# hrbigelow/lb-wavenet

Measured on AMD Instinct MI355X. Metric: audio samples/sec: train fwd+bwd & cached autoregressive gen, 1/2/4/8 GPU, higher is better.
Workload: dtype f32; 1 GPU; C2: train step fwd+xent+bwd+TF1-Adam, par/arch3.json (5x10 layers, res/dil 32, skip/post 512, Q 256), B=8 streams x T=4096 per GPU; arch=arch3.json, batch_per_gpu=8, global_batch=8, slice_sz=4096, parallelism=dp1, world_size_seen=1

## Files before the change

lb-wavenet_amd/csrc/gemm.hip:

```cpp
#include <type_traits>
#include <stdlib.h>
#include <string.h>

#include <algorithm>

#include "common.h"
#include "kernels.h"
#include "prologue.h"

namespace {

constexpr int NT = 256;
constexpr int MNPAD = 8;

template <bool KC, int BMN, int BK>
struct Stage {
  static constexpr int SREG = BK * BMN / (4 * NT);
  static constexpr int KCS = BK + 4;
  static constexpr int RS = BMN + MNPAD;
  floatx4 v[SREG];
  static constexpr int LDS_FLOATS = KC ? BMN * KCS : BK * RS;

  LBWN_DEV void load(const float* __restrict__ P, long ld, int mn0, int MN, int k0, int K, int tid,
                     bool , const int* codes = nullptr) {
// ... 650 lines not shown
        if (g.accumulate) v += cv[r];
      }
      if (row < g.M) {
        if (g.c_chain_ls)
          C[(col >> 5) * g.c_chain_ls + ((((long)(row >> 5) * 4 + ((col >> 3) & 3)) * 32 + (row & 31)) * 8 + (col & 7))] = v;
        else
          C[(long)row * g.ldc + col] = v;
        cs[ni] += v;
      }
    }
  }
  if (g.colpart && !raw) {
    float* red = (float*)smem;
#pragma unroll
    for (int ni = 0; ni < NI; ++ni) {
      cs[ni] += __shfl_xor(cs[ni], 32);
      if (h == 0) red[wave * BN + ni * 32 + ci] = cs[ni];
    }
    __syncthreads();
    const int col = n0 + tid;
    if (tid < BN && col < g.N) {
      float s = 0.f;
      for (int w = 0; w < 8; ++w) s += red[w * BN + tid];
      g.colpart[(long)(m0 >> 8) * g.N + col] = s;
    }
  }
}

template <int CTRL>
LBWN_DEV float quad_xor(float v) {
  return __int_as_float(__builtin_amdgcn_update_dpp(0, __float_as_int(v), CTRL, 0xF, 0xF, true));
}

template <int NB, bool AMN = false, bool KL = false>
__global__ __launch_bounds__(512, 1) void gemm_x3q_kernel(lbwn_gemm_args g) {
  static_assert(!KL || AMN, "k_live: the weight-gradient form");
  constexpr int NP = NB == 10 ? 5 : 2;
  constexpr int NTHR = 512, BM = 256, BN = 16 * NB, NH = NB / NP;
  constexpr int SLOT = BN * X3Q_ROW;
  __shared__ __attribute__((aligned(16))) unsigned short smem[2 * SLOT];

  const int tid = threadIdx.x, lane = tid & 63, wave = tid >> 6;
  const int tiles_n = (g.N + BN - 1) / BN;
  if (g.step_advance && blockIdx.x == 0 && blockIdx.y == 0 && blockIdx.z == 0 && tid == 0)
    __hip_atomic_fetch_add(g.step_advance, 1LL, __ATOMIC_RELAXED, __HIP_MEMORY_SCOPE_AGENT);
  const int t = (NB == 10 && g.xcd2d) ? xcd2d_tile((g.M + BM - 1) / BM, tiles_n) : gemm_tile();
  const int m0 = (t / tiles_n) * BM, n0 = (t % tiles_n) * BN;
  const long mw = ((long)t * 8 + wave) * 64 + lane;
  constexpr bool MB = NB == 8 && !AMN;
  const bool bits_in = MB && g.split_stride == 0 && g.mbits, bits_out = MB && g.split_stride == 0 && g.mbits_out;
  const unsigned long long mbr = bits_in ? g.mbits[mw] : 0ull;
  const int kz0 = KL ? 0 : gemm_split() * g.k_per_split;
  const int kz1 = min(g.K, kz0 + g.k_per_split);
  const LiveSlice ls = KL ? live_slice(g) : LiveSlice{0, 0};
  const int* kl = g.k_live + ls.first;
  const bool dead = !AMN && g.row_live && live_ld(g.row_live + (m0 >> 8)) == 0;
  const int ntiles = KL ? ls.n : (dead ? 0 : (kz1 - kz0) / X3_BK);
  const int last = max(ntiles - 1, 0);
  auto kidx = [&](int i) { return KL ? live_ld(kl + i) : i; };

  floatx4 acc[2][NB];
#pragma unroll
  for (int a = 0; a < 2; ++a)
#pragma unroll
    for (int b = 0; b < NB; ++b) acc[a][b] = (floatx4){0.f, 0.f, 0.f, 0.f};

  const int fr = lane & 15, fq = lane >> 4;
  const long aks = g.a_kstride ? g.a_kstride : X3_BK;
  const int ag0 = min(m0 + 32 * wave, max((g.M - 1) & ~31, 0));
  const float* pa0 = AMN ? (g.a_gstride ? g.A + (ag0 >> 5) * g.a_gstride + fr + (long)(kz0 + 8 * fq) * 32
                                        : g.A + min(m0 + 32 * wave + fr, g.M - 1) + (long)(kz0 + 8 * fq) * g.lda)
                         : g.A + (long)min(m0 + 32 * wave + fr, g.M - 1) * g.lda + (kz0 / X3_BK) * aks + 8 * fq;
  const float* pa1 = AMN ? (g.a_gstride ? pa0 + 16
// ... 3 lines not shown
  floatx4 av[2][4];
  auto a_load = [&](auto sset, int kt) {
    constexpr int S = decltype(sset)::value;
    if (AMN) {
      const long ko = (long)kt * X3_BK * g.lda;
#pragma unroll
      for (int j = 0; j < 8; ++j) {
        av[S][j >> 2][j & 3] = pa0[ko + j * g.lda];
        av[S][2 + (j >> 2)][j & 3] = pa1[ko + j * g.lda];
      }
    } else if (NB == 10) {
      av[S][0] = __builtin_nontemporal_load((const floatx4*)(pa0 + kt * aks));
      av[S][1] = __builtin_nontemporal_load((const floatx4*)(pa0 + kt * aks + 4));
      av[S][2] = __builtin_nontemporal_load((const floatx4*)(pa1 + kt * aks));
      av[S][3] = __builtin_nontemporal_load((const floatx4*)(pa1 + kt * aks + 4));
    } else {
      av[S][0] = *(const floatx4*)(pa0 + kt * aks);
      av[S][1] = *(const floatx4*)(pa0 + kt * aks + 4);
      av[S][2] = *(const floatx4*)(pa1 + kt * aks);
      av[S][3] = *(const floatx4*)(pa1 + kt * aks + 4);
    }
  };
  auto a_split = [&](auto sset, int mi, bf16x8 (&f)[3]) {
    constexpr int S = decltype(sset)::value;
    floatx4 x = av[S][2 * mi], y = av[S][2 * mi + 1];
#pragma unroll
    for (int j = 0; j < 4; ++j) {
      x[j] = __int_as_float(max(__float_as_int(x[j]), alo));
      y[j] = __int_as_float(max(__float_as_int(y[j]), alo));
    }
    split8(x, y, f);
  };

  X3Pre<BN, NTHR, X3Q_ROW> sp;
  X3Stage<false, true, BN, NTHR, X3Q_ROW> sm_b;
  auto b_load = [&](auto sset, int kt) {
    constexpr int S = decltype(sset)::value;
    if (AMN) sm_b.template load<S>(kt, 0);
    else sp.template load<S>(kt);
  };
  auto b_store = [&](auto sset, unsigned short* lds) {
    constexpr int S = decltype(sset)::value;
    if (AMN) sm_b.template store<S>(lds, tid, false);
    else sp.template store<S>(lds);
  };
  if (AMN) sm_b.init(g.B, g.ldb, n0, g.N, kz0, tid);
  else sp.init(g.b3, g.K / X3_BK, n0, g.N, kz0, tid);
  int kn = 0;
  if (ntiles > 0) {
    const int k0 = kidx(0), k1 = kidx(min(1, last)), k2 = kidx(min(2, last));
    if (KL) kn = kidx(min(3, last));
    b_load(std::integral_constant<int, 0>(), k0);
    b_store(std::integral_constant<int, 0>(), smem);
    a_load(std::integral_constant<int, 0>(), k0);
    a_load(std::integral_constant<int, 1>(), k1);
    b_load(std::integral_constant<int, 1>(), k1);
    b_load(std::integral_constant<int, 0>(), k2);
  }
  __syncthreads();
  const int fb_off = fr * X3Q_ROW + 8 * fq;

  auto b_frags = [&](const unsigned short* base, int half, bf16x8 (&f)[NH][3]) {
#pragma unroll
    for (int p = 0; p < 3; ++p)
#pragma unroll
      for (int nb = 0; nb < NH; ++nb) f[nb][p] = *(const bf16x8*)(base + fb_off + (NH * half + nb) * 16 * X3Q_ROW + 32 * p);
  };
  auto mfmas = [&](const bf16x8 (&fa)[2][3], const bf16x8 (&fb)[NH][3], int half) {
#pragma unroll
    for (int qq = 0; qq < 6; ++qq) {
      constexpr int PA[6] = {2, 1, 0, 1, 0, 0}, PB[6] = {0, 1, 2, 0, 1, 0};
#pragma unroll
      for (int mi = 0; mi < 2; ++mi)
#pragma unroll
        for (int nb = 0; nb < NH; ++nb)
          acc[mi][NH * half + nb] =
              __builtin_amdgcn_mfma_f32_16x16x32_bf16(fa[mi][PA[qq]], fb[nb][PB[qq]], acc[mi][NH * half + nb], 0, 0, 0);
    }
  };
  bf16x8 fa[2][3];
  auto step = [&](int kt, auto sset) {
    constexpr int S = decltype(sset)::value;
    const unsigned short* cur = smem + (S ^ 1) * SLOT;
    unsigned short* nxt = smem + S * SLOT;
    bf16x8 fn[2][3], fb[NH][3];
    b_frags(cur, 0, fb);
    mfmas(fa, fb, 0);
    a_split(std::integral_constant<int, S>(), 0, fn[0]);
    a_split(std::integral_constant<int, S>(), 1, fn[1]);
    const int k3 = KL ? kn : min(kt + 3, last);
    a_load(std::integral_constant<int, S>(), k3);
    b_store(std::integral_constant<int, S>(), nxt);
    b_load(std::integral_constant<int, S>(), k3);
    if (KL) kn = live_ld(kl + min(kt + 4, last));
#pragma unroll
    for (int part = 1; part < NP; ++part) {
      b_frags(cur, part, fb);
      mfmas(fa, fb, part);
    }
#pragma unroll
    for (int c = 0; c < 2; ++c)
#pragma unroll
      for (int p = 0; p < 3; ++p) fa[c][p] = fn[c][p];
    __syncthreads();
  };
  if (ntiles > 0) {
    a_split(std::integral_constant<int, 0>(), 0, fa[0]);
    a_split(std::integral_constant<int, 0>(), 1, fa[1]);
    a_load(std::integral_constant<int, 0>(), kidx(min(2, last)));
  }
  int kt = 0;
  for (; kt + 1 < ntiles; kt += 2) {
    step(kt, std::integral_constant<int, 1>());
    step(kt + 1, std::integral_constant<int, 0>());
  }
  if (kt < ntiles) step(kt, std::integral_constant<int, 1>());

  float* C = g.C + (long)gemm_split() * g.split_stride;
  const bool raw = g.split_stride != 0;
  const int rbase = m0 + 32 * wave;
  float cs[NB];
  if (g.c_chain_ls && !raw) {
#pragma unroll
    for (int nb = 0; nb < NB; ++nb) {
      cs[nb] = 0.f;
      const int col0 = n0 + nb * 16;
      if (col0 >= g.N) continue;
      const long chunk = g.c_chain_ls * 4;
      const __amdgpu_buffer_rsrc_t rc = __builtin_amdgcn_make_buffer_rsrc(
          C + (long)(col0 >> 5) * g.c_chain_ls, (short)0, (int)(chunk < 0x7fffffffL ? chunk : 0x7fffffffL), 0x00020000);
      const int c = fr & 3, colq = col0 + 4 * (fr >> 2);
#pragma unroll
      for (int mi = 0; mi < 2; ++mi) {
        float a0 = acc[mi][nb][0], a1 = acc[mi][nb][1], a2 = acc[mi][nb][2], a3 = acc[mi][nb][3];
#pragma unroll
        for (int e = 0; e < 4; ++e)
          if (rbase + 16 * mi + 4 * fq + e < g.M) cs[nb] += acc[mi][nb][e];
        const bool odd = c & 1, hi = c & 2;
        {
          const float r0 = quad_xor<0xB1>(odd ? a0 : a1), r1 = quad_xor<0xB1>(odd ? a2 : a3);
          if (odd) { a0 = r0; a2 = r1; } else { a1 = r0; a3 = r1; }
        }
        {
          const float q0 = quad_xor<0x4E>(hi ? a0 : a2), q1 = quad_xor<0x4E>(hi ? a1 : a3);
          if (hi) { a0 = q0; a1 = q1; } else { a2 = q0; a3 = q1; }
        }
        const int row = rbase + 16 * mi + 4 * fq + c;
        const int off = row < g.M ? (int)(((((long)(row >> 5) * 4 + ((colq >> 3) & 3)) * 32 + (row & 31)) * 8 + (colq & 7)) * 4)
                                  : 0x7ffffff0;
// ... 82 lines not shown
        if (g.accumulate) v += cv[e];
      }
      if (col >= g.N) continue;
      if (row < g.M) {
        if (g.c_chain_ls)
          C[(col >> 5) * g.c_chain_ls + ((((long)(row >> 5) * 4 + ((col >> 3) & 3)) * 32 + (row & 31)) * 8 + (col & 7))] = v;
        else
          C[(long)row * g.ldc + col] = v;
        cs[nb] += v;
      }
    }
  }
  if (bits_out) g.mbits_out[mw] = mbw;
  }
  if (g.colpart && !raw) {
    float* red = (float*)smem;
#pragma unroll
    for (int nb = 0; nb < NB; ++nb) {
      cs[nb] += __shfl_xor(cs[nb], 16);
      cs[nb] += __shfl_xor(cs[nb], 32);
      if (fq == 0) red[wave * BN + nb * 16 + fr] = cs[nb];
    }
    __syncthreads();
    const int col = n0 + tid;
    if (tid < BN && col < g.N) {
      float s = 0.f;
      for (int w = 0; w < 8; ++w) s += red[w * BN + tid];
      g.colpart[(long)(m0 >> 8) * g.N + col] = s;
    }
  }
}

static_assert(PLANE_BK == X3_BK, "pre-split chunk = GEMM k-step");
__global__ void split_planes_kernel(SplitJobs jb) { split_planes_body(jb, blockIdx.y, blockIdx.x, gridDim.x); }

}

namespace {
thread_local const char* g_last_form = "";

int gemm_setup(const lbwn_gemm_args& a, int a_kcontig, int b_kcontig, int& split_k, float* slab_ws, int BK,
               int BM, int BN, lbwn_gemm_args& g, dim3& grid) {
  LBWN_REQUIRE(a.M > 0 && a.N > 0 && a.K > 0, "gemm: empty shape M=%d N=%d K=%d", a.M, a.N, a.K);
  LBWN_REQUIRE(a.K % 4 == 0 || !a_kcontig, "gemm: K %% 4 != 0 with k-contiguous A");
  LBWN_REQUIRE(a.K % 4 == 0 || !b_kcontig, "gemm: K %% 4 != 0 with k-contiguous B");
  LBWN_REQUIRE(a.M % 4 == 0 || a_kcontig, "gemm: M %% 4 != 0 with m-contiguous A");
  LBWN_REQUIRE(a.N % 4 == 0, "gemm: N %% 4 != 0");
  LBWN_REQUIRE(a.lda % 4 == 0 && a.ldb % 4 == 0, "gemm: lda/ldb must be multiples of 4");
  LBWN_REQUIRE(a.a_codes == nullptr || !a_kcontig, "gemm: one-hot A must be m-contiguous");
  LBWN_REQUIRE((a.a_codes || (((uintptr_t)a.A) & 15) == 0) && (((uintptr_t)a.B) & 15) == 0,
               "gemm: A/B not 16-B aligned");
  LBWN_REQUIRE(!a.a_kstride || (a_kcontig && a.lda == 32 && a.K % 32 == 0 && !a.a_codes && lbwn_gemm_mode() == 1),
               "gemm: k-blocked A needs k-contiguous A, lda = 32, K %% 32 == 0 and the bf16-split form");
  LBWN_REQUIRE(!a.b_gstride || (!b_kcontig && a.ldb == 32 && !a.b3 && lbwn_gemm_mode() == 1),
               "gemm: mn-blocked B needs mn-contiguous B, ldb = 32, no pre-split and the bf16-split form");
  LBWN_REQUIRE(!a.a_gstride || (!a_kcontig && a.lda == 32 && !b_kcontig && !a.b_gstride && !a.b3 && a.M >= 256 &&
                                a.K % 32 == 0 && !a.mask && !a.bias && !a.colpart && !a.c_chain_ls && !a.a_codes &&
                                lbwn_gemm_mode() == 1),
               "gemm: mn-blocked A needs the AMN weight-gradient form (lda = 32, M >= 256, K %% 32 == 0)");
  LBWN_REQUIRE(!a.splits_deferred || (!a.bias && !a.relu_out && !a.mask && !a.accumulate),
               "gemm: deferred split-K needs a plain product");
  if (split_k < 1) split_k = 1;
  g = a;
  int kps = (a.K + split_k - 1) / split_k;
  kps = (kps + BK - 1) / BK * BK;
  split_k = (a.K + kps - 1) / kps;
  g.k_per_split = kps;
// ... 65 lines not shown
                   !(X3Q && X3R && a_kcontig && a.b3 && (a.colpart || (a.N <= 2048 && (a.M >= 8192 || a.row_exact)))),
               "gemm (bf16 split): chain-order C on the A-in-registers form (gemm_x3q_kernel) takes no bias / relu_out / "
               "mask bits");
  LBWN_REQUIRE(!(a.mbits || a.mbits_out) ||
                   (lbwn_gemm_x3q8_form(a.M, a.N, a.K, a_kcontig, a.b3 != nullptr, a.row_exact, a.colpart != nullptr) &&
                    split_k <= 1),
               "gemm (bf16 split): mask bits need the gemm_x3q_kernel<8> form without split-K");
  LBWN_REQUIRE(!a.row_live || (lbwn_gemm_row_live_form(a.M, a.N, a.K, a_kcontig, a.b3 != nullptr, a.row_exact,
                                                       a.colpart != nullptr) && split_k <= 1),
               "gemm (bf16 split): row_live needs the k-contiguous gemm_x3q_kernel<8 / 10> form without split-K");
  const bool klist = a.k_live || a.nk_live || a.k_pre;
  LBWN_REQUIRE(!klist || (a.k_live && a.nk_live && a.k_pre && !a_kcontig && !b_kcontig && !a.b3 && !a.a_gstride && !a.b_gstride &&
                          !a.colpart && !a.c_chain_ls && lbwn_gemm_k_live_form(a.M, a.N, a.K)),
               "gemm (bf16 split): k_live needs a plain mn-contiguous weight-gradient product with K %% 32 == 0");
  const int wm = (a.colpart || (a_kcontig && a.N <= 2048 && (a.M >= 8192 || a.row_exact))) ? 4 : 2;
  lbwn_gemm_args g;
  dim3 grid;
  int e = gemm_setup(a, a_kcontig, b_kcontig, split_k, slab_ws, X3_BK, 64 * wm, 128, g, grid);
  if (e) return e;
  const bool kfull = a.K % X3_BK == 0, pre = a.b3 != nullptr;
  if (X3Q && !a_kcontig && !b_kcontig && kfull && !pre && !a.mask && !a.bias && !a.colpart && !a.c_chain_ls &&
      !a.b_gstride && a.M >= 256 && a.N % 4 == 0 && (((a.M + 255) / 256) * ((a.N + 127) / 128) >= 8 || a.a_gstride)) {
    if ((e = gemm_setup(a, a_kcontig, b_kcontig, split_k, slab_ws, X3_BK, 256, a.N <= 96 ? 96 : 128, g, grid))) return e;
    g_last_form = a.N <= 96 ? "x3q<6,amn>" : klist ? "x3q<8,amn,kl>" : "x3q<8,amn>";
    if (a.N <= 96) gemm_x3q_kernel<6, true><<<grid, 512, 0, st>>>(g);
    else if (klist) gemm_x3q_kernel<8, true, true><<<grid, 512, 0, st>>>(g);
    else gemm_x3q_kernel<8, true><<<grid, 512, 0, st>>>(g);
    LBWN_CHECK_LAUNCH();
    return splitk_finish(a, split_k, slab_ws, st);
  }
  LBWN_REQUIRE(!a.a_gstride, "gemm: mn-blocked A (a_gstride) needs the AMN A-in-registers form (X3Q, no pre-split B, "
                             "no epilogue, M >= 256)");
  if (wm == 4 && X3R && kfull && pre && a_kcontig) {
    if (a.N <= 96) {
      grid.x = (unsigned)(((a.M + 255) / 256) * ((a.N + 95) / 96));
      g_last_form = X3Q ? "x3q<6>" : "x3r<3>";
      if (X3Q) gemm_x3q_kernel<6><<<grid, 512, 0, st>>>(g);
      else gemm_x3r_kernel<3><<<grid, 512, 0, st>>>(g);
    } else if (X3Q && a.N % 160 == 0 && a.N > 512) {
      grid.x = (unsigned)(((a.M + 255) / 256) * (a.N / 160));
      g_last_form = "x3q<10>";
      gemm_x3q_kernel<10><<<grid, 512, 0, st>>>(g);
    } else if (X3Q) {
      g_last_form = "x3q<8>";
      gemm_x3q_kernel<8><<<grid, 512, 0, st>>>(g);
    } else {
      g_last_form = "x3r<4>";
      gemm_x3r_kernel<4><<<grid, 512, 0, st>>>(g);
    }
    LBWN_CHECK_LAUNCH();
  } else if (wm == 4) {
    if (kfull && pre) e = gemm_launch_x3_t<true, true, 4>(g, grid, a_kcontig, b_kcontig, st);
    else if (kfull) e = gemm_launch_x3_t<true, false, 4>(g, grid, a_kcontig, b_kcontig, st);
    else e = gemm_launch_x3_t<false, false, 4>(g, grid, a_kcontig, b_kcontig, st);
  } else if (klist) {
    g_last_form = "x3<kl>";
    gemm_x3_kernel<false, false, true, false, 2, 1, true><<<grid, 256, 0, st>>>(g);
    LBWN_CHECK_LAUNCH();
  } else {
    if (kfull && pre) e = gemm_launch_x3_t<true, true, 2>(g, grid, a_kcontig, b_kcontig, st);
    else if (kfull) e = gemm_launch_x3_t<true, false, 2>(g, grid, a_kcontig, b_kcontig, st);
    else e = gemm_launch_x3_t<false, false, 2>(g, grid, a_kcontig, b_kcontig, st);
  }
  if (e) return e;
  return splitk_finish(a, split_k, slab_ws, st);
}

template <int BK, int BMT, int BNT>
int gemm_launch_t(const lbwn_gemm_args& a, int a_kcontig, int b_kcontig, int split_k, float* slab_ws, hipStream_t st) {
  lbwn_gemm_args g;
  dim3 grid;
  int e = gemm_setup(a, a_kcontig, b_kcontig, split_k, slab_ws, BK, BMT, BNT, g, grid);
  if (e) return e;
  g_last_form = a_kcontig ? (b_kcontig ? "f32<akc,bkc>" : "f32<akc,bmn>") : (b_kcontig ? "f32<amn,bkc>" : "f32<amn,bmn>");
  if (a_kcontig && b_kcontig) gemm_f32_kernel<true, true, BK, BMT, BNT><<<grid, NT, 0, st>>>(g);
  else if (a_kcontig) gemm_f32_kernel<true, false, BK, BMT, BNT><<<grid, NT, 0, st>>>(g);
  else if (b_kcontig) gemm_f32_kernel<false, true, BK, BMT, BNT><<<grid, NT, 0, st>>>(g);
  else gemm_f32_kernel<false, false, BK, BMT, BNT><<<grid, NT, 0, st>>>(g);
// ... 68 lines not shown
```

lb-wavenet_amd/csrc/engine.cpp:

```cpp
#include <stdio.h>
#include <stdlib.h>
#include <string.h>

#include <algorithm>
#include <new>

#include "../../include/lbwn.h"
#include "common.h"
#include "kernels.h"

struct lbwn_plan {
  int chain_xcd = 0;
  int dz_xcd2d = 1;
  int fwd_mode = -1;
  int ncu = 0;
  size_t oMBS = 0, oMBR = 0;
  bool mb_s = false, mb_r = false;
  bool mbits_ok = true;
  size_t oLIVE = 0;
  bool skip_ok = true;
  bool live_valid = false;
  bool dv_blk = false;
  bool dz_blk = false;
  int head_colparts = 0;
// ... 415 lines not shown
    p->oPADG = carve(cur, sizeof(float) * hp);
  }
  p->total = cur;
  *out = p;
  return 0;
}

void lbwn_plan_destroy(lbwn_plan* p) { delete p; }

int lbwn_plan_tensor(const lbwn_plan* p, const char* name, size_t* off, size_t* bytes) {
  LBWN_REQUIRE(p && name && off && bytes, "plan_tensor: null argument");
  const size_t M = (size_t)p->M, f = sizeof(float);
  if (!strcmp(name, "x")) { *off = p->oX; *bytes = f * (size_t)p->x_layer_stride * p->L; }
  else if (!strcmp(name, "z")) { *off = p->oZ; *bytes = f * M * p->L * p->Cd; }
  else if (!strcmp(name, "s")) { *off = p->oS; *bytes = f * M * p->Cs; }
  else if (!strcmp(name, "r2")) { *off = p->oR2; *bytes = f * M * p->Cp; }
  else if (!strcmp(name, "logits")) { *off = p->oLOG; *bytes = f * M * p->Q; }
  else if (!strcmp(name, "status")) { *off = p->oSTATUS; *bytes = 16; }
  else if (!strcmp(name, "ctrace")) { *off = p->oCTRACE; *bytes = 8 * 2 * 16 * (size_t)p->a.n_blocks * p->a.n_block_layers; }
  else if (!strcmp(name, "dh")) { *off = p->oDH; *bytes = f * M * p->Cp; }
  else if (!strcmp(name, "ds")) { *off = p->oDS; *bytes = f * M * p->Cs; }
  else if (!strcmp(name, "dz")) { *off = p->oDZ; *bytes = f * (p->dz_blk ? (size_t)m32(p->M) : M) * p->L * p->Cd; }
  else if (!strcmp(name, "tlive")) { *off = p->oLIVE; *bytes = 4 * ((M + 255) / 256); }
  else if (!strcmp(name, "klive")) { *off = p->oLIVE + 4 * ((M + 255) / 256); *bytes = 4 * ((M + 31) / 32); }
  else if (!strcmp(name, "nklive")) { *off = p->oLIVE + 4 * ((M + 255) / 256 + (M + 31) / 32); *bytes = 4; }
  else if (!strcmp(name, "kpre")) { *off = p->oLIVE + 4 * ((M + 255) / 256 + (M + 31) / 32 + 1); *bytes = 4 * ((M + 31) / 32 + 1); }
  else if (!strcmp(name, "cond") && p->Lo) { *off = p->oCOND; *bytes = f * M * 2 * p->L * p->Cd; }
  else if (!strcmp(name, "dvall") && p->Lo) {
    *off = p->oDVALL;
    *bytes = f * (p->dv_blk ? (size_t)m32(p->M) : M) * 2 * p->L * p->Cd;
  }
  else if (!strcmp(name, "gctab") && p->Ge) { *off = p->oGCTAB; *bytes = f * p->ncat1 * 2 * p->L * p->Cd; }
  else if (!strcmp(name, "gcd") && p->Ge) { *off = p->oGCD; *bytes = f * p->ncat1 * 2 * p->L * p->Cd; }
  else LBWN_REQUIRE(false, "plan_tensor: unknown tensor '%s'", name);
  return 0;
}
size_t lbwn_plan_workspace_bytes(const lbwn_plan* p) { return p ? p->total : 0; }

int lbwn_plan_info(const lbwn_plan* p, const char* key, int64_t* value) {
  LBWN_REQUIRE(p && key && value, "plan_info: null argument");
  if (!strcmp(key, "up_fused")) *value = p->up_fused;
  else if (!strcmp(key, "up_fused_bwd")) *value = p->up_fused_bwd;
  else if (!strcmp(key, "lc_in_chain")) *value = p->oLCX != 0 && p->chain;
  else if (!strcmp(key, "split_dlc")) *value = p->split_dlc;
  else if (!strcmp(key, "split_dlcx")) *value = p->split_dlcx;
  else if (!strcmp(key, "split_dlct")) *value = p->split_dlct;
  else if (!strncmp(key, "split_up", 8) && key[8] >= '0' && key[8] <= '7' && !key[9])
    *value = p->split_up[key[8] - '0'];
  else if (!strcmp(key, "dv_blk")) *value = p->dv_blk;
  else if (!strcmp(key, "dlc_parts")) *value = p->dlc_parts;
  else if (!strcmp(key, "dmel_fused")) *value = p->dmel_fused;
  else LBWN_REQUIRE(false, "plan_info: unknown key '%s'", key);
  return 0;
}

static int* live_t(const lbwn_plan* p, void* ws) { return reinterpret_cast<int*>(static_cast<char*>(ws) + p->oLIVE); }
static int* live_k(const lbwn_plan* p, void* ws) { return live_t(p, ws) + (p->M + 255) / 256; }
static int* live_n(const lbwn_plan* p, void* ws) { return live_k(p, ws) + (p->M + 31) / 32; }
static int* live_p(const lbwn_plan* p, void* ws) { return live_n(p, ws) + 1; }

static const unsigned short* w3(const lbwn_plan* p, void* ws, int i) {
  return (p->oW3[i] && lbwn_gemm_mode() == 1) ? reinterpret_cast<const unsigned short*>(static_cast<char*>(ws) + p->oW3[i])
                                              : nullptr;
}

static lbwn_gemm_args gemm0() {
// ... 745 lines not shown
```

lb-wavenet_amd/csrc/pack.hip:

```cpp
#include <string.h>

#include "common.h"
#include "kernels.h"
#include "layer_common.h"
#include "prologue.h"

namespace {


__global__ void pack_layers_kernel(const float* sig, const float* gate, const float* sig_b, const float* gate_b,
                                   const float* res, const float* res_b, float* out, int Cr, int Cd) {
  const int l = blockIdx.x;
  const float* ws = sig + (long)l * 2 * Cr * Cd;
  const float* wg = gate + (long)l * 2 * Cr * Cd;
  const float* wr = res + (long)l * Cd * Cr;
  float* img = out + (long)l * WIMG;
  for (int e = threadIdx.x; e < 64 * WS; e += blockDim.x) {
    const int k = e / WS, o = e % WS;
    const int tap = k >> 5, in = k & 31, oc = o & 31;
    float v = 0.f;
    if (o < 64 && in < Cr && oc < Cd) v = (o < 32 ? ws : wg)[(tap * Cr + in) * Cd + oc];
    img[e] = v;
  }
  for (int e = threadIdx.x; e < 32 * XS; e += blockDim.x) {
// ... 165 lines not shown
  const int nlc = lcout ? L : 0;
  if (l < L) {
    pack_x3_body(l, sig, gate, sig_b, gate_b, res, res_b, fout, Cr, Cd);
  } else if (l < 2 * L) {
    pack_bx3_body(l - L, sig, gate, res, bout, Cr, Cd);
  } else if (l < 2 * L + nlc) {
    if (lc16) pack_lc16_body(l - 2 * L, lc_sig, lc_gate, lcout, Lo, Cd);
    else pack_lc_x3_body(l - 2 * L, lc_sig, lc_gate, lcout, Lo, Cd);
  } else {
    const int n = (l - 2 * L - nlc) * 256 + threadIdx.x;
    if (n < Cs) {
      float s = 0.f;
#pragma unroll 10
      for (int k = 0; k < L; ++k) s += skip_b[(long)k * Cs + n];
      bsum[n] = s;
    }
  }
}
__global__ __launch_bounds__(256) void pack_layers_fb_x3_kernel(const float* sig, const float* gate,
                                                                const float* sig_b, const float* gate_b,
                                                                const float* res, const float* res_b,
                                                                unsigned short* fout, float* bout, int L, int Cr,
                                                                int Cd, const float* skip_b, int Cs, float* bsum,
                                                                const float* lc_sig, const float* lc_gate, int Lo,
                                                                unsigned short* lcout, int lc16) {
  pack_fb_x3_block(blockIdx.x, sig, gate, sig_b, gate_b, res, res_b, fout, bout, L, Cr, Cd, skip_b, Cs, bsum, lc_sig,
                   lc_gate, Lo, lcout, lc16);
}

struct PrologueK {
  lbwn_prologue_args a;
  SplitJobs jb;
  int nz, ns, ne, nd, np;
  int nl;
  bool ev4, dv4;
};
__global__ __launch_bounds__(256) void step_prologue_kernel(PrologueK k) {
  const lbwn_prologue_args& a = k.a;
  long b = blockIdx.x;
  if (b < k.nl) {
    live_lists_body(a.ids, a.B, a.T, a.tlive, a.klive, a.nklive, a.kpre);
    return;
  }
  b -= k.nl;
  if (b < (long)k.ns * a.njobs) {
    split_planes_body(k.jb, (int)(b / k.ns), b % k.ns, k.ns);
    return;
  }
  b -= (long)k.ns * a.njobs;
  if (b < k.ne) {
    embed_flat_body(b, k.ne, a.q, a.pre, a.pre_b, a.X, a.B, a.T, a.H, a.Cr, a.Q, k.ev4);
    return;
  }
  b -= k.ne;
  if (b < k.nd) {
    dsep_flat_body<true>(b, k.nd, a.X, a.xls, const_cast<float*>(a.save), a.L, a.nbl, a.B, a.T, a.H, a.Cr, k.dv4);
    return;
  }
  b -= k.nd;
  if (b < k.nz) {
    zero_body(b, k.nz, (unsigned*)a.zero, (long)(a.zero_bytes / 4));
    return;
  }
  b -= k.nz;
  pack_fb_x3_block((int)b, a.sig, a.gate, a.sig_b, a.gate_b, a.res, a.res_b, a.fout, a.bout, a.L, a.Cr, a.Cd,
                   a.skip_b, a.Cs, a.bsum, a.lc_sig, a.lc_gate, a.Lo, a.lcout, a.lc16);
}

}

int lbwn_layer_image_floats() { return WIMG; }
int lbwn_layer_image_x3_elems() { return XIMG_US; }
int lbwn_lc_image_x3_elems() { return LCIMG_US; }
int lbwn_lc_image16_elems() { return LC16IMG_US; }
int lbwn_lc_in_chain_ok(int Lo) { return Lo > 16 * (LC_K - 1) && Lo <= LC_KP && Lo % 4 == 0; }
int lbwn_layer_image_bx3_floats() { return BIMG_F; }

int lbwn_pack_layers_launch(const float* sig, const float* gate, const float* sig_b, const float* gate_b,
                            const float* res, const float* res_b, float* out, int L, int Cr, int Cd, hipStream_t st) {
  pack_layers_kernel<<<L, 256, 0, st>>>(sig, gate, sig_b, gate_b, res, res_b, out, Cr, Cd);
  LBWN_CHECK_LAUNCH();
  return 0;
}

int lbwn_pack_layers_fb_x3_launch(const float* sig, const float* gate, const float* sig_b, const float* gate_b,
                                  const float* res, const float* res_b, unsigned short* fout, float* bout, int L,
                                  int Cr, int Cd, const float* skip_b, int Cs, float* bsum, const float* lc_sig,
                                  const float* lc_gate, int Lo, unsigned short* lcout, hipStream_t st, int lc16) {
  LBWN_REQUIRE(Cr <= 32 && Cd <= 32 && (((uintptr_t)fout) & 15) == 0 && (((uintptr_t)bout) & 15) == 0,
               "pack_layers_fb_x3: bad arguments");
  LBWN_REQUIRE(!lcout || (lc_sig && lc_gate && Lo >= 1 && Lo <= LC_KP && (((uintptr_t)lcout) & 15) == 0),
               "pack_layers_fb_x3: bad LC image arguments");
  const int nsum = (skip_b && bsum) ? (Cs + 255) / 256 : 0;
  const int nlc = lcout ? L : 0;
  pack_layers_fb_x3_kernel<<<2 * L + nlc + nsum, 256, 0, st>>>(sig, gate, sig_b, gate_b, res, res_b, fout, bout, L, Cr,
                                                               Cd, skip_b, Cs, bsum, lc_sig, lc_gate, Lo, lcout,
                                                               lc16);
  LBWN_CHECK_LAUNCH();
  return 0;
}
int lbwn_step_prologue_launch(const lbwn_prologue_args& a, hipStream_t st) {
  LBWN_REQUIRE(a.Cr <= 32 && a.Cd <= 32 && (((uintptr_t)a.fout) & 15) == 0 && (((uintptr_t)a.bout) & 15) == 0,
               "step_prologue: bad pack arguments");
  LBWN_REQUIRE(!a.lcout || (a.lc_sig && a.lc_gate && a.Lo >= 1 && a.Lo <= LC_KP && (((uintptr_t)a.lcout) & 15) == 0),
               "step_prologue: bad LC image arguments");
  LBWN_REQUIRE(a.njobs >= 0 && a.njobs <= 6 && a.zero_bytes % 4 == 0 && a.q && a.pre && a.X && a.save,
               "step_prologue: bad arguments");
  PrologueK k;
  memset(&k, 0, sizeof(k));
  k.a = a;
  long most = 0;
  for (int j = 0; j < a.njobs; ++j) {
    LBWN_REQUIRE(a.W[j] && a.out[j] && a.rows[j] > 0 && a.K[j] > 0, "step_prologue: bad split job");
    k.jb.W[j] = a.W[j]; k.jb.ldw[j] = a.ldw[j]; k.jb.rows[j] = a.rows[j]; k.jb.K[j] = a.K[j];
    k.jb.trans[j] = a.trans[j]; k.jb.out[j] = a.out[j];
    most = std::max(most, (long)a.rows[j] * ((a.K[j] + PLANE_BK - 1) / PLANE_BK) * (PLANE_BK / 2));
  }
  auto blocks = [](long n, long per, long cap) { return (int)std::max(1L, std::min(cap, (n + per - 1) / per)); };
  k.ns = blocks(most, 1024, 256);
  LBWN_REQUIRE((long)a.B * a.T * a.Cr < (1L << 31) && (long)dsep_rows(a.L, a.nbl, 1) * a.B * a.Cr < (1L << 31),
               "step_prologue: x / SAVE exceed 32-bit indexing");
  k.ev4 = embed_v4(a.pre, a.pre_b, a.X, a.Cr);
  k.dv4 = dsep_v4(a.X, a.xls, a.save, a.Cr);
  k.ne = blocks((long)a.B * a.T * (k.ev4 ? a.Cr / 4 : a.Cr), 256, 2048);
  k.nd = blocks((long)dsep_rows(a.L, a.nbl, a.B) * (k.dv4 ? a.Cr / 4 : a.Cr), 256, 2048);
  k.nz = a.zero_bytes ? blocks((long)(a.zero_bytes / 4), 1024, 256) : 0;
  k.np = 2 * a.L + (a.lcout ? a.L : 0) + ((a.skip_b && a.bsum) ? (a.Cs + 255) / 256 : 0);
  LBWN_REQUIRE(!a.ids || (a.tlive && a.klive && a.nklive && a.kpre), "step_prologue: bad live-list arguments");
  k.nl = a.ids ? 1 : 0;
  const long grid = (long)k.nl + (long)k.ns * a.njobs + k.ne + k.nd + k.nz + k.np;
  step_prologue_kernel<<<(unsigned)grid, 256, 0, st>>>(k);
  LBWN_CHECK_LAUNCH();
  return 0;
}
```

lb-wavenet_amd/csrc/prologue.h:

```cpp
#pragma once
#include "common.h"

constexpr int PLANE_BK = 32;

__host__ __device__ inline int dsep_rows(int L, int nbl, int B) {
  return ((L / nbl) * ((1 << nbl) - 1) + ((1 << (L % nbl)) - 1)) * B;
}

template <bool TO_X>
LBWN_DEV void dsep_flat_body(long blk, long nblk, float* xall, long xls, float* save, int L, int nbl, int B, int T,
                             int H, int Cr, bool v4) {
  const int per = (1 << nbl) - 1, rows = dsep_rows(L, nbl, B);
  const int cw = v4 ? Cr >> 2 : Cr;
  const int n = rows * cw;
  for (int e = (int)(blk * 256) + (int)threadIdx.x; e < n; e += (int)(nblk * 256)) {
    const int R = e / cw, c = e - R * cw;
    const int run = R / (B * per), w = R - run * (B * per);
    const int k = 31 - __builtin_clz(w / B + 1);
    const int local = w - B * ((1 << k) - 1);
    const int b = local >> k, i = local & ((1 << k) - 1), d = 1 << k;
    float* xr = xall + (long)(run * nbl + k) * xls + ((long)b * (H + T) + (TO_X ? H - d + i : H + T - d + i)) * Cr;
    float* sv = save + (long)R * Cr;
    if (v4) {
      if (TO_X) *(floatx4*)(xr + 4 * c) = *(const floatx4*)(sv + 4 * c);
// ... 9 lines not shown
inline bool dsep_v4(const float* xall, long xls, const float* save, int Cr) {
  return (Cr & 3) == 0 && (xls & 3) == 0 && al16(xall) && al16(save);
}
inline bool embed_v4(const float* pre, const float* pre_b, const float* x0, int Cr) {
  return (Cr & 3) == 0 && al16(pre) && (!pre_b || al16(pre_b)) && al16(x0);
}

LBWN_DEV void embed_flat_body(long blk, long nblk, const int* __restrict__ q, const float* __restrict__ pre,
                              const float* pre_b, float* x0, int B, int T, int H, int Cr, int Q, bool v4) {
  const int cw = v4 ? Cr >> 2 : Cr;
  const int n = B * T * cw;
  for (int e = (int)(blk * 256) + (int)threadIdx.x; e < n; e += (int)(nblk * 256)) {
    const int m = e / cw, c = e - m * cw;
    const int b = m / T, t = m - b * T;
    int code = q[m];
    code = code < 0 ? 0 : (code >= Q ? Q - 1 : code);
    float* xo = x0 + ((long)b * (H + T) + H + t) * Cr;
    if (v4) {
      floatx4 v = *(const floatx4*)(pre + (long)code * Cr + 4 * c);
      if (pre_b) v += *(const floatx4*)(pre_b + 4 * c);
      *(floatx4*)(xo + 4 * c) = v;
    } else {
      float v = pre[(long)code * Cr + c];
      if (pre_b) v += pre_b[c];
      xo[c] = v;
    }
  }
}

LBWN_DEV void zero_body(long blk, long nblk, unsigned* p, long n) {
  for (long e = blk * 256 + threadIdx.x; e < n; e += nblk * 256) p[e] = 0u;
}

LBWN_DEV void live_lists_body(const int* __restrict__ ids, int B, int T, int* tlive, int* klive, int* nklive,
                              int* kpre) {
  __shared__ int wcnt[4];
  const int M = B * T, nk = (M + 31) / 32, nt = (M + 255) / 256;
  const int tid = threadIdx.x, lane = tid & 63, w = tid >> 6;
  const int inc = 64 % T;
  constexpr int NL = 16, KW = 2 * NL, KR = 4 * KW;
  auto row0 = [&](int k0) { return 32 * (k0 + KW * w) + lane; };
  int v[NL], nx[NL];
  auto load = [&](int (&d)[NL], int k0) {
#pragma unroll
    for (int j = 0; j < NL; ++j) d[j] = ids[min(row0(k0) + 64 * j + 1, M - 1)];
  };
  load(v, 0);
  int base = 0;
  for (int k0 = 0; k0 < nk; k0 += KR) {
    load(nx, min(k0 + KR, nk));
    const int r0 = row0(k0);
    int t = r0 % T;
    unsigned live = 0u;
#pragma unroll
    for (int j = 0; j < NL; ++j) {
      const unsigned long long bal = __ballot((r0 + 64 * j < M) & (t != T - 1) & (v[j] != 0));
      live |= (unsigned)((unsigned)bal != 0u) << (2 * j);
      live |= (unsigned)((bal >> 32) != 0ull) << (2 * j + 1);
      t += inc;
      t -= t >= T ? T : 0;
    }
    const int k = k0 + KW * w + lane;
    if (lane == 0) wcnt[w] = __popc(live);
    __syncthreads();
    int off = base, tot = 0;
#pragma unroll
    for (int i = 0; i < 4; ++i) {
      off += i < w ? wcnt[i] : 0;
      tot += wcnt[i];
    }
    const int pos = off + __popc(live & ((1u << (lane & 31)) - 1u));
    if (lane < KW && k < nk) kpre[k] = pos;
    if (lane < KW && ((live >> lane) & 1u)) klive[pos] = k;
    if (lane < KW && (lane & 7) == 0 && (k >> 3) < nt) tlive[k >> 3] = ((live >> lane) & 0xffu) != 0u;
    base += tot;
    __syncthreads();
#pragma unroll
    for (int j = 0; j < NL; ++j) v[j] = nx[j];
  }
  if (tid == 0) {
    *nklive = base;
    kpre[nk] = base;
  }
}

struct SplitJobs {
  const float* W[6];
  long ldw[6];
  int rows[6], K[6], trans[6];
  unsigned short* out[6];
};
LBWN_DEV void split_planes_body(const SplitJobs& jb, int jj, long blk, long nblk) {
  const float* __restrict__ W = jb.W[jj];
  const long ldw = jb.ldw[jj];
  const int rows = jb.rows[jj], K = jb.K[jj], trans = jb.trans[jj];
  unsigned short* __restrict__ out = jb.out[jj];
  const int kch = (K + PLANE_BK - 1) / PLANE_BK;
  const long total = (long)rows * kch * (PLANE_BK / 2);
  for (long e = blk * 256 + threadIdx.x; e < total; e += nblk * 256) {
    const int j2 = (int)(e % (PLANE_BK / 2)) * 2;
    const long rc = e / (PLANE_BK / 2);
    const int kc = (int)(rc % kch), r = (int)(rc / kch);
    const int k = kc * PLANE_BK + j2;
    floatx2 x;
    x[0] = k < K ? (trans ? W[(long)k * ldw + r] : W[(long)r * ldw + k]) : 0.f;
    x[1] = k + 1 < K ? (trans ? W[(long)(k + 1) * ldw + r] : W[(long)r * ldw + k + 1]) : 0.f;
    unsigned h, m, l;
    split2(x, h, m, l);
    unsigned* o = (unsigned*)(out + rc * (3 * PLANE_BK) + j2);
    o[0] = h;
    o[PLANE_BK / 2] = m;
    o[PLANE_BK] = l;
  }
}
```

Measured before the change: 17.86 million audio samples/s.

## Load pre-split B tiles via global_load_lds DMA with four-slot LDS ring

Adds a DMA variant of the x3q GEMM kernel in which B tiles are copied straight from global memory into LDS with global_load_lds_dwordx4, bypassing the register-staged load/store path. It uses a four-slot LDS ring, issues DMA for two tiles ahead every other step, and replaces per-step __syncthreads with explicit vmcnt/lgkmcnt waits plus a barrier every two steps. The goal is to cut VGPR pressure and store instructions for B and to overlap loads with MFMA work. This DMA variant is now the default for the NB=8 pre-split path and opt-in via env var for the NB=6 and NB=10 paths. It doubles LDS use and depends on hand-written waitcnt counts being exact.

After: 17.90 million audio samples/s (median of 3 runs). About the same (+0.2%).

```diff
diff --git a/lb-wavenet_amd/csrc/gemm.hip b/lb-wavenet_amd/csrc/gemm.hip
--- a/lb-wavenet_amd/csrc/gemm.hip
+++ b/lb-wavenet_amd/csrc/gemm.hip
@@ -706,13 +706,23 @@
   return __int_as_float(__builtin_amdgcn_update_dpp(0, __float_as_int(v), CTRL, 0xF, 0xF, true));
 }
 
-template <int NB, bool AMN = false, bool KL = false>
+LBWN_DEV void x3q_dma16(const unsigned short* sbase, unsigned voff, unsigned lds_dst) {
+  unsigned saved;
+  asm volatile("s_mov_b32 %0, m0\n\ts_mov_b32 m0, %1\n\ts_nop 0\n\tglobal_load_lds_dwordx4 %2, %3\n\ts_mov_b32 m0, %0"
+               : "=&s"(saved)
+               : "s"(lds_dst), "v"(voff), "s"(sbase)
+               : "memory");
+}
+
+template <int NB, bool AMN = false, bool KL = false, bool DMA = false>
 __global__ __launch_bounds__(512, 1) void gemm_x3q_kernel(lbwn_gemm_args g) {
   static_assert(!KL || AMN, "k_live: the weight-gradient form");
+  static_assert(!DMA || !AMN, "B by LDS-DMA: the pre-split k-contiguous forms");
   constexpr int NP = NB == 10 ? 5 : 2;
   constexpr int NTHR = 512, BM = 256, BN = 16 * NB, NH = NB / NP;
   constexpr int SLOT = BN * X3Q_ROW;
-  __shared__ __attribute__((aligned(16))) unsigned short smem[2 * SLOT];
+  constexpr int NSLOT = DMA ? 4 : 2;
+  __shared__ __attribute__((aligned(16))) unsigned short smem[NSLOT * SLOT];
 
   const int tid = threadIdx.x, lane = tid & 63, wave = tid >> 6;
   const int tiles_n = (g.N + BN - 1) / BN;
@@ -782,6 +792,29 @@
     split8(x, y, f);
   };
 
+  constexpr int NPIECE = BN * 14 / 64, PW = (NPIECE + 7) / 8;
+  static_assert((BN * 14) % 64 == 0, "B by LDS-DMA: whole 1-KiB pieces");
+  const int wv = __builtin_amdgcn_readfirstlane(wave);
+  unsigned dvoff[PW];
+  const unsigned short* dbase = nullptr;
+  unsigned ddst = 0;
+  if (DMA) {
+    const int kchunks = g.K / X3_BK;
+#pragma unroll
+    for (int i = 0; i < PW; ++i) {
+      const int gi = min(wv + 8 * i, NPIECE - 1) * 64 + lane, r = gi / 14, part = gi % 14;
+      dvoff[i] = (unsigned)(((long)min(n0 + r, g.N - 1) * kchunks * (3 * X3_BK) + 8 * (part < 12 ? part : 0)) * 2);
+    }
+    dbase = g.b3 + (long)(kz0 / X3_BK) * (3 * X3_BK);
+    ddst = (unsigned)(uintptr_t)(__attribute__((address_space(3))) unsigned short*)smem + wv * 1024;
+  }
+  auto b_dma = [&](int kt) {
+    const unsigned short* sb = dbase + (long)min(kt, last) * (3 * X3_BK);
+    const unsigned dst = ddst + (kt & 3) * (SLOT * 2);
+#pragma unroll
+    for (int i = 0; i < PW; ++i) x3q_dma16(sb, dvoff[i], dst + min(8 * i, NPIECE - 1 - wv) * 1024);
+  };
+
   X3Pre<BN, NTHR, X3Q_ROW> sp;
   X3Stage<false, true, BN, NTHR, X3Q_ROW> sm_b;
   auto b_load = [&](auto sset, int kt) {
@@ -795,9 +828,17 @@
     else sp.template store<S>(lds);
   };
   if (AMN) sm_b.init(g.B, g.ldb, n0, g.N, kz0, tid);
-  else sp.init(g.b3, g.K / X3_BK, n0, g.N, kz0, tid);
+  else if (!DMA) sp.init(g.b3, g.K / X3_BK, n0, g.N, kz0, tid);
   int kn = 0;
-  if (ntiles > 0) {
+  if (DMA) {
+    if (ntiles > 0) {
+      b_dma(0);
+      b_dma(1);
+      a_load(std::integral_constant<int, 0>(), 0);
+      a_load(std::integral_constant<int, 1>(), min(1, last));
+    }
+    asm volatile("s_waitcnt vmcnt(8)\n\ts_waitcnt lgkmcnt(0)\n\ts_barrier" ::: "memory");
+  } else if (ntiles > 0) {
     const int k0 = kidx(0), k1 = kidx(min(1, last)), k2 = kidx(min(2, last));
     if (KL) kn = kidx(min(3, last));
     b_load(std::integral_constant<int, 0>(), k0);
@@ -807,7 +848,7 @@
     b_load(std::integral_constant<int, 1>(), k1);
     b_load(std::integral_constant<int, 0>(), k2);
   }
-  __syncthreads();
+  if (!DMA) __syncthreads();
   const int fb_off = fr * X3Q_ROW + 8 * fq;
 
   auto b_frags = [&](const unsigned short* base, int half, bf16x8 (&f)[NH][3]) {
@@ -831,28 +872,51 @@
   bf16x8 fa[2][3];
   auto step = [&](int kt, auto sset) {
     constexpr int S = decltype(sset)::value;
-    const unsigned short* cur = smem + (S ^ 1) * SLOT;
+    const unsigned short* cur = smem + (DMA ? (kt & 3) : (S ^ 1)) * SLOT;
     unsigned short* nxt = smem + S * SLOT;
     bf16x8 fn[2][3], fb[NH][3];
+    const int k3 = KL ? kn : min(kt + 3, last);
+    constexpr int PMID = (NP - 1) / 2;
+    auto stage = [&]() {
+      a_split(std::integral_constant<int, S>(), 0, fn[0]);
+      a_split(std::integral_constant<int, S>(), 1, fn[1]);
+      asm volatile("" : "+v"(fn[0][2]), "+v"(fn[1][2]));
+      if (S == 1) {
+        b_dma(kt + 2);
+        b_dma(kt + 3);
+      }
+      a_load(std::integral_constant<int, S>(), k3);
+      asm volatile("" ::: "memory");
+    };
     b_frags(cur, 0, fb);
     mfmas(fa, fb, 0);
-    a_split(std::integral_constant<int, S>(), 0, fn[0]);
-    a_split(std::integral_constant<int, S>(), 1, fn[1]);
-    const int k3 = KL ? kn : min(kt + 3, last);
-    a_load(std::integral_constant<int, S>(), k3);
-    b_store(std::integral_constant<int, S>(), nxt);
-    b_load(std::integral_constant<int, S>(), k3);
+    if (DMA) {
+      if (PMID == 0) stage();
+    } else {
+      a_split(std::integral_constant<int, S>(), 0, fn[0]);
+      a_split(std::integral_constant<int, S>(), 1, fn[1]);
+    }
+    if (!DMA) {
+      a_load(std::integral_constant<int, S>(), k3);
+      b_store(std::integral_constant<int, S>(), nxt);
+      b_load(std::integral_constant<int, S>(), k3);
+    }
     if (KL) kn = live_ld(kl + min(kt + 4, last));
 #pragma unroll
     for (int part = 1; part < NP; ++part) {
       b_frags(cur, part, fb);
       mfmas(fa, fb, part);
+      if (DMA && part == PMID) stage();
     }
 #pragma unroll
     for (int c = 0; c < 2; ++c)
 #pragma unroll
       for (int p = 0; p < 3; ++p) fa[c][p] = fn[c][p];
-    __syncthreads();
+    if (!DMA) {
+      __syncthreads();
+    } else if (S == 0) {
+      asm volatile("s_waitcnt vmcnt(4)\n\ts_waitcnt lgkmcnt(0)\n\ts_barrier" ::: "memory");
+    }
   };
   if (ntiles > 0) {
     a_split(std::integral_constant<int, 0>(), 0, fa[0]);
@@ -865,6 +929,7 @@
     step(kt + 1, std::integral_constant<int, 0>());
   }
   if (kt < ntiles) step(kt, std::integral_constant<int, 1>());
+  if (DMA) asm volatile("s_waitcnt vmcnt(0)\n\ts_waitcnt lgkmcnt(0)\n\ts_barrier" ::: "memory");
 
   float* C = g.C + (long)gemm_split() * g.split_stride;
   const bool raw = g.split_stride != 0;
@@ -1145,18 +1210,23 @@
   LBWN_REQUIRE(!a.a_gstride, "gemm: mn-blocked A (a_gstride) needs the AMN A-in-registers form (X3Q, no pre-split B, "
                              "no epilogue, M >= 256)");
   if (wm == 4 && X3R && kfull && pre && a_kcontig) {
+    const char* bv = getenv("LBWN_GEMM_BDMA");
+    const bool bdma = !(bv && bv[0] == '0'), bdma_opt = bv && bv[0] == '1';
     if (a.N <= 96) {
       grid.x = (unsigned)(((a.M + 255) / 256) * ((a.N + 95) / 96));
-      g_last_form = X3Q ? "x3q<6>" : "x3r<3>";
-      if (X3Q) gemm_x3q_kernel<6><<<grid, 512, 0, st>>>(g);
+      g_last_form = X3Q ? (bdma_opt ? "x3q<6,bdma>" : "x3q<6>") : "x3r<3>";
+      if (X3Q && bdma_opt) gemm_x3q_kernel<6, false, false, true><<<grid, 512, 0, st>>>(g);
+      else if (X3Q) gemm_x3q_kernel<6><<<grid, 512, 0, st>>>(g);
       else gemm_x3r_kernel<3><<<grid, 512, 0, st>>>(g);
     } else if (X3Q && a.N % 160 == 0 && a.N > 512) {
       grid.x = (unsigned)(((a.M + 255) / 256) * (a.N / 160));
-      g_last_form = "x3q<10>";
-      gemm_x3q_kernel<10><<<grid, 512, 0, st>>>(g);
+      g_last_form = bdma_opt ? "x3q<10,bdma>" : "x3q<10>";
+      if (bdma_opt) gemm_x3q_kernel<10, false, false, true><<<grid, 512, 0, st>>>(g);
+      else gemm_x3q_kernel<10><<<grid, 512, 0, st>>>(g);
     } else if (X3Q) {
-      g_last_form = "x3q<8>";
-      gemm_x3q_kernel<8><<<grid, 512, 0, st>>>(g);
+      g_last_form = bdma ? "x3q<8>" : "x3q<8,breg>";
+      if (bdma) gemm_x3q_kernel<8, false, false, true><<<grid, 512, 0, st>>>(g);
+      else gemm_x3q_kernel<8><<<grid, 512, 0, st>>>(g);
     } else {
       g_last_form = "x3r<4>";
       gemm_x3r_kernel<4><<<grid, 512, 0, st>>>(g);
```

## Tile transposed weight plane-split through LDS and widen live-list scan

Applied to the files above, without the earlier changes.

Transposed weight jobs in the per-step plane-split now stage a 64-row by one-k-chunk tile through shared memory, so reads from W stay coalesced instead of striding by ldw. Each split job gets its own block count, and the combined prologue grid is the sum of those counts rather than a uniform max times the job count. The live-list scan now reads four ids per lane in a single vector load and packs one 64-bit flag word per wave, so it uses fewer ballots. Embed and dsep get fewer, larger blocks. The cost is extra shared memory and barriers in the prologue kernel and more complex boundary handling in the live-list scan.

Measured after the change: 17.68 million audio samples/s before, 17.71 million audio samples/s after, median of 3. No clear change (+0.1%).

```diff
diff --git a/lb-wavenet_amd/csrc/engine.cpp b/lb-wavenet_amd/csrc/engine.cpp
--- a/lb-wavenet_amd/csrc/engine.cpp
+++ b/lb-wavenet_amd/csrc/engine.cpp
@@ -471,6 +471,11 @@
   }
   else if (!strcmp(name, "gctab") && p->Ge) { *off = p->oGCTAB; *bytes = f * p->ncat1 * 2 * p->L * p->Cd; }
   else if (!strcmp(name, "gcd") && p->Ge) { *off = p->oGCD; *bytes = f * p->ncat1 * 2 * p->L * p->Cd; }
+  else if (!strncmp(name, "w3_", 3) && name[3] >= '0' && name[3] <= '5' && !name[4] && p->oW3[name[3] - '0']) {
+    const W3Shape w = w3_shape(p, name[3] - '0');
+    *off = p->oW3[name[3] - '0'];
+    *bytes = 2 * lbwn_split_planes_elems(w.rows, w.K);
+  }
   else LBWN_REQUIRE(false, "plan_tensor: unknown tensor '%s'", name);
   return 0;
 }
diff --git a/lb-wavenet_amd/csrc/gemm.hip b/lb-wavenet_amd/csrc/gemm.hip
--- a/lb-wavenet_amd/csrc/gemm.hip
+++ b/lb-wavenet_amd/csrc/gemm.hip
@@ -1013,7 +1013,9 @@
 }
 
 static_assert(PLANE_BK == X3_BK, "pre-split chunk = GEMM k-step");
-__global__ void split_planes_kernel(SplitJobs jb) { split_planes_body(jb, blockIdx.y, blockIdx.x, gridDim.x); }
+__global__ __launch_bounds__(256) void split_planes_kernel(SplitJobs jb) {
+  split_planes_body(jb, blockIdx.y, blockIdx.x, gridDim.x);
+}
 
 }
 
diff --git a/lb-wavenet_amd/csrc/pack.hip b/lb-wavenet_amd/csrc/pack.hip
--- a/lb-wavenet_amd/csrc/pack.hip
+++ b/lb-wavenet_amd/csrc/pack.hip
@@ -221,6 +221,7 @@
   lbwn_prologue_args a;
   SplitJobs jb;
   int nz, ns, ne, nd, np;
+  int nsj[6];
   int nl;
   bool ev4, dv4;
 };
@@ -232,11 +233,13 @@
     return;
   }
   b -= k.nl;
-  if (b < (long)k.ns * a.njobs) {
-    split_planes_body(k.jb, (int)(b / k.ns), b % k.ns, k.ns);
-    return;
-  }
-  b -= (long)k.ns * a.njobs;
+  if (b < k.ns) {
+    int j = 0;
+    while (b >= k.nsj[j]) b -= k.nsj[j++];
+    split_planes_body(k.jb, j, b, k.nsj[j]);
+    return;
+  }
+  b -= k.ns;
   if (b < k.ne) {
     embed_flat_body(b, k.ne, a.q, a.pre, a.pre_b, a.X, a.B, a.T, a.H, a.Cr, a.Q, k.ev4);
     return;
@@ -298,26 +301,27 @@
   PrologueK k;
   memset(&k, 0, sizeof(k));
   k.a = a;
-  long most = 0;
+  auto blocks = [](long n, long per, long cap) { return (int)std::max(1L, std::min(cap, (n + per - 1) / per)); };
   for (int j = 0; j < a.njobs; ++j) {
     LBWN_REQUIRE(a.W[j] && a.out[j] && a.rows[j] > 0 && a.K[j] > 0, "step_prologue: bad split job");
     k.jb.W[j] = a.W[j]; k.jb.ldw[j] = a.ldw[j]; k.jb.rows[j] = a.rows[j]; k.jb.K[j] = a.K[j];
     k.jb.trans[j] = a.trans[j]; k.jb.out[j] = a.out[j];
-    most = std::max(most, (long)a.rows[j] * ((a.K[j] + PLANE_BK - 1) / PLANE_BK) * (PLANE_BK / 2));
-  }
-  auto blocks = [](long n, long per, long cap) { return (int)std::max(1L, std::min(cap, (n + per - 1) / per)); };
-  k.ns = blocks(most, 1024, 256);
+    k.nsj[j] = a.trans[j] ? blocks(split_planes_tiles(a.rows[j], a.K[j]), 2, 512)
+                          : blocks((long)a.rows[j] * ((a.K[j] + PLANE_BK - 1) / PLANE_BK) * (PLANE_BK / 2), 2048, 512);
+    k.ns += k.nsj[j];
+  }
   LBWN_REQUIRE((long)a.B * a.T * a.Cr < (1L << 31) && (long)dsep_rows(a.L, a.nbl, 1) * a.B * a.Cr < (1L << 31),
                "step_prologue: x / SAVE exceed 32-bit indexing");
   k.ev4 = embed_v4(a.pre, a.pre_b, a.X, a.Cr);
   k.dv4 = dsep_v4(a.X, a.xls, a.save, a.Cr);
-  k.ne = blocks((long)a.B * a.T * (k.ev4 ? a.Cr / 4 : a.Cr), 256, 2048);
-  k.nd = blocks((long)dsep_rows(a.L, a.nbl, a.B) * (k.dv4 ? a.Cr / 4 : a.Cr), 256, 2048);
+  k.ne = blocks((long)a.B * a.T * (k.ev4 ? a.Cr / 4 : a.Cr), 1024, 2048);
+  k.nd = blocks((long)dsep_rows(a.L, a.nbl, a.B) * (k.dv4 ? a.Cr / 4 : a.Cr), 1024, 2048);
   k.nz = a.zero_bytes ? blocks((long)(a.zero_bytes / 4), 1024, 256) : 0;
   k.np = 2 * a.L + (a.lcout ? a.L : 0) + ((a.skip_b && a.bsum) ? (a.Cs + 255) / 256 : 0);
-  LBWN_REQUIRE(!a.ids || (a.tlive && a.klive && a.nklive && a.kpre), "step_prologue: bad live-list arguments");
+  LBWN_REQUIRE(!a.ids || (a.tlive && a.klive && a.nklive && a.kpre && (long)a.B * a.T >= 4),
+               "step_prologue: bad live-list arguments");
   k.nl = a.ids ? 1 : 0;
-  const long grid = (long)k.nl + (long)k.ns * a.njobs + k.ne + k.nd + k.nz + k.np;
+  const long grid = (long)k.nl + k.ns + k.ne + k.nd + k.nz + k.np;
   step_prologue_kernel<<<(unsigned)grid, 256, 0, st>>>(k);
   LBWN_CHECK_LAUNCH();
   return 0;
diff --git a/lb-wavenet_amd/csrc/prologue.h b/lb-wavenet_amd/csrc/prologue.h
--- a/lb-wavenet_amd/csrc/prologue.h
+++ b/lb-wavenet_amd/csrc/prologue.h
@@ -65,36 +65,57 @@
   for (long e = blk * 256 + threadIdx.x; e < n; e += nblk * 256) p[e] = 0u;
 }
 
+struct __attribute__((packed, aligned(4))) IdsX4 { int v[4]; };
+LBWN_DEV unsigned nonzero_bytes(unsigned long long x) {
+  x |= x >> 4;
+  x |= x >> 2;
+  x |= x >> 1;
+  return (unsigned)(((x & 0x0101010101010101ull) * 0x0102040810204080ull) >> 56);
+}
 LBWN_DEV void live_lists_body(const int* __restrict__ ids, int B, int T, int* tlive, int* klive, int* nklive,
                               int* kpre) {
   __shared__ int wcnt[4];
   const int M = B * T, nk = (M + 31) / 32, nt = (M + 255) / 256;
-  const int tid = threadIdx.x, lane = tid & 63, w = tid >> 6;
-  const int inc = 64 % T;
-  constexpr int NL = 16, KW = 2 * NL, KR = 4 * KW;
-  auto row0 = [&](int k0) { return 32 * (k0 + KW * w) + lane; };
-  int v[NL], nx[NL];
-  auto load = [&](int (&d)[NL], int k0) {
-#pragma unroll
-    for (int j = 0; j < NL; ++j) d[j] = ids[min(row0(k0) + 64 * j + 1, M - 1)];
-  };
-  load(v, 0);
+  const int tid = threadIdx.x, lane = tid & 63, w = __builtin_amdgcn_readfirstlane(tid >> 6);
+  const int inc = 256 % T;
+  constexpr int NL = 8, KW = 8 * NL, KR = 4 * KW;
+  static_assert(KW == 64, "a wave's flags are one 64-bit word, a k-step per lane");
+  auto row0 = [&](int k0) { return 32 * (k0 + KW * w) + 4 * lane; };
+  auto first = [&](int r) { return min(r + 1, M - 4); };
+  IdsX4 v[NL];
   int base = 0;
   for (int k0 = 0; k0 < nk; k0 += KR) {
-    load(nx, min(k0 + KR, nk));
     const int r0 = row0(k0);
+#pragma unroll
+    for (int j = 0; j < NL; ++j) v[j] = *(const IdsX4*)(ids + first(r0 + 256 * j));
     int t = r0 % T;
-    unsigned live = 0u;
+    unsigned long long live = 0ull;
+    const bool inner = T >= 4 && 32 * (k0 + KW * w) + 256 * NL + 1 <= M;
 #pragma unroll
     for (int j = 0; j < NL; ++j) {
-      const unsigned long long bal = __ballot((r0 + 64 * j < M) & (t != T - 1) & (v[j] != 0));
-      live |= (unsigned)((unsigned)bal != 0u) << (2 * j);
-      live |= (unsigned)((bal >> 32) != 0ull) << (2 * j + 1);
+      bool any = false;
+      if (inner) {
+        const int ex = T - 1 - t;
+        any = ((v[j].v[0] != 0) & (ex != 0)) | ((v[j].v[1] != 0) & (ex != 1)) | ((v[j].v[2] != 0) & (ex != 2)) |
+              ((v[j].v[3] != 0) & (ex != 3));
+      } else {
+        const int r = r0 + 256 * j, sh = r + 1 - first(r);
+        int te = t;
+#pragma unroll
+        for (int e = 0; e < 4; ++e) {
+          int id = 0;
+#pragma unroll
+          for (int q = 0; q < 4; ++q) id = e + sh == q ? v[j].v[q] : id;
+          any |= (r + e < M) & (te != T - 1) & (id != 0);
+          te = te + 1 == T ? 0 : te + 1;
+        }
+      }
+      live |= (unsigned long long)nonzero_bytes(__ballot(any)) << (8 * j);
       t += inc;
       t -= t >= T ? T : 0;
     }
     const int k = k0 + KW * w + lane;
-    if (lane == 0) wcnt[w] = __popc(live);
+    if (lane == 0) wcnt[w] = __popcll(live);
     __syncthreads();
     int off = base, tot = 0;
 #pragma unroll
@@ -102,14 +123,12 @@
       off += i < w ? wcnt[i] : 0;
       tot += wcnt[i];
     }
-    const int pos = off + __popc(live & ((1u << (lane & 31)) - 1u));
-    if (lane < KW && k < nk) kpre[k] = pos;
-    if (lane < KW && ((live >> lane) & 1u)) klive[pos] = k;
-    if (lane < KW && (lane & 7) == 0 && (k >> 3) < nt) tlive[k >> 3] = ((live >> lane) & 0xffu) != 0u;
+    const int pos = off + __popcll(live & ((1ull << lane) - 1ull));
+    if (k < nk) kpre[k] = pos;
+    if ((live >> lane) & 1ull) klive[pos] = k;
+    if ((lane & 7) == 0 && (k >> 3) < nt) tlive[k >> 3] = ((live >> lane) & 0xffull) != 0ull;
     base += tot;
     __syncthreads();
-#pragma unroll
-    for (int j = 0; j < NL; ++j) v[j] = nx[j];
   }
   if (tid == 0) {
     *nklive = base;
@@ -123,11 +142,56 @@
   int rows[6], K[6], trans[6];
   unsigned short* out[6];
 };
+constexpr int SPLIT_TR = 64;
+static_assert(256 % SPLIT_TR == 0 && (PLANE_BK * SPLIT_TR) % 256 == 0,
+              "a tile is whole passes of a 256-thread block");
+__host__ __device__ inline long split_planes_tiles(int rows, int K) {
+  return (long)((rows + SPLIT_TR - 1) / SPLIT_TR) * ((K + PLANE_BK - 1) / PLANE_BK);
+}
+LBWN_DEV void split_planes_trans_body(const float* __restrict__ W, long ldw, int rows, int K,
+                                      unsigned short* __restrict__ out, long blk, long nblk) {
+  __shared__ float tile[PLANE_BK][SPLIT_TR + 1];
+  const int kch = (K + PLANE_BK - 1) / PLANE_BK;
+  const long ntiles = split_planes_tiles(rows, K);
+  const int tid = threadIdx.x;
+  for (long t = blk; t < ntiles; t += nblk) {
+    const int kc = (int)(t % kch), r0 = (int)(t / kch) * SPLIT_TR;
+    {
+      const int rl = tid & (SPLIT_TR - 1), r = r0 + rl;
+#pragma unroll
+      for (int p = 0; p < PLANE_BK * SPLIT_TR / 256; ++p) {
+        const int kl = tid / SPLIT_TR + p * (256 / SPLIT_TR), k = kc * PLANE_BK + kl;
+        tile[kl][rl] = (k < K && r < rows) ? W[(long)k * ldw + r] : 0.f;
+      }
+    }
+    __syncthreads();
+#pragma unroll
+    for (int p = 0; p < SPLIT_TR * (PLANE_BK / 2) / 256; ++p) {
+      const int i = tid + 256 * p, j2 = (i & (PLANE_BK / 2 - 1)) * 2, rl = i / (PLANE_BK / 2), r = r0 + rl;
+      if (r < rows) {
+        floatx2 x;
+        x[0] = tile[j2][rl];
+        x[1] = tile[j2 + 1][rl];
+        unsigned h, m, l;
+        split2(x, h, m, l);
+        unsigned* o = (unsigned*)(out + ((long)r * kch + kc) * (3 * PLANE_BK) + j2);
+        o[0] = h;
+        o[PLANE_BK / 2] = m;
+        o[PLANE_BK] = l;
+      }
+    }
+    __syncthreads();
+  }
+}
 LBWN_DEV void split_planes_body(const SplitJobs& jb, int jj, long blk, long nblk) {
   const float* __restrict__ W = jb.W[jj];
   const long ldw = jb.ldw[jj];
   const int rows = jb.rows[jj], K = jb.K[jj], trans = jb.trans[jj];
   unsigned short* __restrict__ out = jb.out[jj];
+  if (trans) {
+    split_planes_trans_body(W, ldw, rows, K, out, blk, nblk);
+    return;
+  }
   const int kch = (K + PLANE_BK - 1) / PLANE_BK;
   const long total = (long)rows * kch * (PLANE_BK / 2);
   for (long e = blk * 256 + threadIdx.x; e < total; e += nblk * 256) {
@@ -136,8 +200,8 @@
     const int kc = (int)(rc % kch), r = (int)(rc / kch);
     const int k = kc * PLANE_BK + j2;
     floatx2 x;
-    x[0] = k < K ? (trans ? W[(long)k * ldw + r] : W[(long)r * ldw + k]) : 0.f;
-    x[1] = k + 1 < K ? (trans ? W[(long)(k + 1) * ldw + r] : W[(long)r * ldw + k + 1]) : 0.f;
+    x[0] = k < K ? W[(long)r * ldw + k] : 0.f;
+    x[1] = k + 1 < K ? W[(long)r * ldw + k + 1] : 0.f;
     unsigned h, m, l;
     split2(x, h, m, l);
     unsigned* o = (unsigned*)(out + rc * (3 * PLANE_BK) + j2);
```
